# Epist/omnidirectional_collaborative_filtering

Measured on AMD Instinct MI355X. Metric: ratings/sec + masked-RMSE, ML-20M I-AutoRec at 1/2/4/8 MI355X, higher is better.
Workload: dtype f16

## Files before the change

include/ocf.h:

```cpp
#ifndef OCF_H_
#define OCF_H_
#include <stdint.h>

#ifdef __cplusplus
extern "C" {
#endif

#define OCF_DT_F32 0
#define OCF_DT_F16 1
#define OCF_DT_BF16 2

#define OCF_ACTV_LINEAR 0
#define OCF_ACTV_SIGMOID 1
#define OCF_ACTV_TANH 2
#define OCF_ACTV_RELU 3

#define OCF_OPTK_SGD 0
#define OCF_OPTK_ADAGRAD 1
#define OCF_OPTK_RMSPROP 2
#define OCF_OPTK_ADAM 3

#define OCF_EPI_SLAB 0
#define OCF_EPI_BIAS_ACT 1
#define OCF_EPI_GRAD_ACT 2
// ... 253 lines not shown
typedef struct OcfOptStepArgs {
  float* p; const void* g; int g_dtype; float* s1; float* s2; int64_t n; OcfOptParams opt;
  void* shadow; int shadow_dtype;
} OcfOptStepArgs;
int ocf_opt_step_ex(const OcfOptStepArgs* args, void* stream);

int ocf_bias_opt_from_partials(float* b, const float* db_part, int parts, int64_t ld, int n, float* s1, float* s2,
                               float* g_out, const OcfOptParams* opt, void* stream);

int ocf_sumsq(const float* x, int64_t n, float scale, float* ws, float* out, void* stream);

int ocf_stats_finalize(const float* stats_part, int n_parts, const float* row_sse_part, int n_tiles, int M,
                       float* out, void* stream);

#define OCF_LIVE_REC 144

typedef struct OcfTileBucketArgs {
  const int32_t* rows; const int64_t* rp; const int32_t* tptr; const int32_t* col; const int32_t* lidx;
  const int64_t* lboff;
  int krows, ntiles, gm, nk;
  int32_t* cnt; int32_t* bptr; int32_t* ent;
  int64_t cap;
  int counted; int32_t* cnt_clear;
  const uint8_t* rtag_in; const uint8_t* rtag_out; int rtag;
  uint8_t* live_in; uint8_t* live_out;
  int32_t* row_ptr; int32_t* row_ent;
} OcfTileBucketArgs;
int ocf_sparse_tiles(const OcfTileBucketArgs* args, void* stream);

typedef struct OcfRowListArgs {
  const int32_t* ecb; int64_t E;
  int32_t* col_cnt; int32_t* cursor; int n_cols;
  int32_t* row_ptr; int32_t* row_ent;
  const uint8_t* rtag_in; const uint8_t* rtag_out; int rtag;
  uint8_t* live_in; uint8_t* live_out;
} OcfRowListArgs;
int ocf_row_lists(const OcfRowListArgs* args, void* stream);

typedef struct OcfEpochRowListArgs {
  int n_sel; int B; int n_cols;
  const int32_t* rows;
  const int64_t* rp; const int32_t* col;
  const int64_t* lboff;
  const int32_t* sel;
  const int64_t* ebase;
  int32_t* cnt;
  int32_t* row_ptr;
  int32_t* row_ent;
  uint8_t* live;
  int n_rg;
  int64_t ebase0;
  int max_list;
  int64_t entries;
} OcfEpochRowListArgs;
int ocf_epoch_row_lists(const OcfEpochRowListArgs* args, void* stream);

typedef struct OcfRecipKeepArgs {
  uint32_t key[624]; int32_t pos;
  int32_t nb; int32_t B; int64_t n_entries;
  const int64_t* boff; const int64_t* ebase;
  double s0; double s1;
  uint8_t* keep;
  double* doubles;
  void* workspace; int64_t workspace_bytes;
} OcfRecipKeepArgs;
int64_t ocf_recip_keep_workspace(int nb, int B, int64_t n_entries, int pos);
int ocf_recip_keep(OcfRecipKeepArgs* args, void* stream);
int ocf_mt_host_random_sample(uint32_t* key, int32_t* pos, int64_t n, double* out);
int ocf_mt_host_jump(const uint32_t* key_in, int64_t n_blocks, uint32_t* key_out);

#define OCF_MAX_HIDDEN 8
typedef struct OcfModelDesc {
  int n_hidden;
  int N;
  int k_blocks;
  int hidden[OCF_MAX_HIDDEN];
  int act;
  float dropout;
  int compute_dtype;
  int max_batch;
  uint64_t seed;
  float* W[OCF_MAX_HIDDEN + 1];
  float* b[OCF_MAX_HIDDEN + 1];
} OcfModelDesc;
typedef struct OcfCtx OcfCtx;

int ocf_model_dims(const OcfModelDesc* desc, int64_t* rows, int64_t* cols);
int ocf_ctx_create(const OcfModelDesc* desc, OcfCtx** ctx);
int ocf_ctx_destroy(OcfCtx* ctx);
int ocf_forward(OcfCtx* ctx, const float* const* inputs, int64_t ld_in, int B, int training, uint64_t step,
                const float* out_mask, int64_t ld_mask, float* pred, int64_t ld_pred, uint8_t* const* masks_out,
                void* stream);
int ocf_masked_mse(const float* pred, const float* T, const float* out_mask, int64_t ld, int B, int N,
                   float* out_grad, int64_t ld_grad, float* out_stats, void* stream);
int ocf_backward(OcfCtx* ctx, const float* grad, int64_t ld_grad, int B, float gscale, float* const* gW,
                 float* const* gb, void* stream);

typedef struct OcfMlpStepArgs {
  int n_hidden;
  int B, Bp;
  int N, Np, k_blocks;
  int hidden[OCF_MAX_HIDDEN], hidden_p[OCF_MAX_HIDDEN];
  const float* x[3]; int64_t ld_x; const int64_t* rows;
  const float* out_mask; const float* targets; int64_t ld_t;
  float* W[OCF_MAX_HIDDEN + 1]; float* b[OCF_MAX_HIDDEN + 1];
  float* sW1[OCF_MAX_HIDDEN + 1]; float* sW2[OCF_MAX_HIDDEN + 1];
// ... 32 lines not shown
```

omnidirectional_collaborative_filtering_amd/_lib.py:

```python
from __future__ import annotations

import ctypes
import os

_HERE = os.path.dirname(os.path.abspath(__file__))
LIB_PATH = os.environ.get("OCF_LIB_PATH") or os.path.join(_HERE, "libocf.so")

DT_F32, DT_F16, DT_BF16 = 0, 1, 2
ACT = {"linear": 0, None: 0, "sigmoid": 1, "tanh": 2, "relu": 3}
OPT_SGD, OPT_ADAGRAD, OPT_RMSPROP, OPT_ADAM = 0, 1, 2, 3
LIVE_REC = 144
EPI_SLAB, EPI_BIAS_ACT, EPI_GRAD_ACT, EPI_GRAD, EPI_OPTIM, EPI_PREDICT, EPI_MASKED_MSE = range(7)

P = ctypes.c_void_p
I32 = ctypes.c_int
I64 = ctypes.c_int64
U64 = ctypes.c_uint64
F32 = ctypes.c_float


class OcfOptParams(ctypes.Structure):
    _fields_ = [("kind", I32), ("lr", F32), ("eps", F32), ("rho", F32), ("beta2", F32), ("l2", F32),
                ("gscale", F32)]


class OcfScatterArgs(ctypes.Structure):
    _fields_ = [
        ("rp1", P), ("col1", P), ("val1", P), ("dup1", P), ("rows1", P), ("keep1", P), ("boff1", P),
        ("s0", F32), ("s1", F32), ("seed", U64), ("stream", U64), ("mode", I32), ("pass_through", I32),
        ("rp2", P), ("col2", P), ("val2", P), ("dup2", P), ("rows2", P),
        ("B", I32), ("B_pad", I32), ("N", I32), ("aux", F32),
        ("X", P), ("Min", P), ("Mout", P), ("T", P), ("Mmiss", P), ("ld", I64),
        ("xin", P), ("xin_dtype", I32), ("xin_ld", I64), ("xin_block", I64), ("feed", I32), ("both", I32),
        ("tile_cnt", P), ("bk_ptr", P), ("bk_cur", P), ("bk_rc", P), ("bk_t", P), ("bk_m", P), ("n_tiles", I32),
        ("pos1", P),
        ("lboff1", P), ("lboff2", P), ("E1", I64), ("E2", I64), ("tflag1", P), ("tflag2", P),
        ("xin_clean", I32), ("xval1", P), ("tb_cnt", P), ("tb_nk", I32),
        ("rtag_in", P), ("rtag_out", P), ("rtag", I32), ("col_cnt", P), ("ecb", P),
    ]


class OcfRowListArgs(ctypes.Structure):
    _fields_ = [
        ("ecb", P), ("E", I64), ("col_cnt", P), ("cursor", P), ("n_cols", I32), ("row_ptr", P), ("row_ent", P),
        ("rtag_in", P), ("rtag_out", P), ("rtag", I32), ("live_in", P), ("live_out", P),
    ]


class OcfEpochScatterArgs(ctypes.Structure):
    _fields_ = [
        ("n_sel", I32), ("sel", P), ("ebase", P), ("max_e", I64), ("keep_off", P), ("stream_mul", U64),
        ("xval", P), ("tflag", P), ("ebase0", I64),
    ]


class OcfEpochRowListArgs(ctypes.Structure):
    _fields_ = [
        ("n_sel", I32), ("B", I32), ("n_cols", I32), ("rows", P), ("rp", P), ("col", P), ("lboff", P),
        ("sel", P), ("ebase", P), ("cnt", P), ("row_ptr", P), ("row_ent", P), ("live", P), ("n_rg", I32),
        ("ebase0", I64), ("max_list", I32), ("entries", I64),
    ]


class OcfEncTileArgs(ctypes.Structure):
    _fields_ = [
        ("rows", P), ("rp", P), ("tptr", P), ("tcol", P), ("tlidx", P), ("lboff", P), ("xval", P),
        ("W", P), ("ldw", I64), ("w_dtype", I32), ("B", I32), ("Bp", I32), ("n_tiles", I32), ("H", I32),
        ("splits", I32), ("part", P), ("nnz", I64), ("n_entries", I64), ("work", P), ("work_bytes", I64),
        ("max_row_len", I64),
    ]


class OcfGatherArgs(ctypes.Structure):
    _fields_ = [
        ("rows", P), ("rp", P), ("col", P), ("val", P), ("lboff", P), ("xval", P), ("flag", P),
        ("ch_row", P), ("ch_j0", P), ("ch_j1", P), ("n_chunks", I32),
        ("W", P), ("w_dtype", I32), ("ldw", I64), ("w_blocked", I32), ("H", I32), ("part", P),
        ("h", P), ("h_dtype", I32), ("bias", P), ("aux", F32), ("delta_e", P), ("chunk_stats", P),
        ("d_out", P), ("d_dtype", I32), ("ld_d", I64),
        ("enc_part", P), ("enc_cptr", P), ("bias_h", P), ("act", I32), ("keep", F32), ("seed", U64), ("stream", U64),
        ("a_out", P), ("mask_out", P), ("m_real", I32), ("n_real", I32), ("zero_word", P),
        ("jr", P), ("row_arrive", P),
    ]


REDUCE_RAW, REDUCE_BIAS_ACT, REDUCE_GRAD_ACT = 0, 1, 2


class OcfRowsReduceArgs(ctypes.Structure):
    _fields_ = [
        ("part", P), ("row_cptr", P), ("B", I32), ("Bp", I32), ("H", I32), ("mode", I32), ("out", P),
        ("bias", P), ("act", I32), ("keep", F32), ("seed", U64), ("stream", U64),
        ("mask_in", P), ("mask_out", P), ("a_out", P), ("a_in", P), ("h_out", P), ("h_dtype", I32), ("n_real", I32),
        ("db_part", P), ("gscale", F32), ("chunk_stats", P), ("stats_part", P), ("row_sse", P),
    ]


class OcfGemmArgs(ctypes.Structure):
    _fields_ = [
        ("compute_dtype", I32),
        ("A", P), ("a_dtype", I32), ("a_col", I32), ("lda", I64),
        ("B", P), ("b_dtype", I32), ("b_col", I32), ("ldb", I64),
        ("M", I32), ("N", I32), ("K", I32), ("splits", I32), ("order", I32), ("epi", I32),
        ("out", P), ("ld_out", I64), ("split_stride", I64),
        ("bias", P), ("act", I32), ("keep", F32), ("seed", U64), ("stream", U64),
        ("mask_in", P), ("mask_out", P), ("a_out", P), ("h_out", P), ("h_dtype", I32), ("a_in", P),
        ("db_part", P), ("ld_db", I64), ("m_real", I32), ("n_real", I32),
        ("p", P), ("s1", P), ("s2", P), ("opt", OcfOptParams),
        ("pmask", P), ("ld_pmask", I64),
        ("bk_ptr", P), ("bk_rc", P), ("bk_t", P), ("bk_m", P), ("stats_part", P), ("row_sse_part", P),
        ("t_rows", P), ("t_rp", P), ("t_tptr", P), ("t_col", P), ("t_val", P), ("t_lidx", P), ("t_flag", P),
        ("t_lboff", P), ("t_ntiles", I32), ("t_aux", F32),
        ("p_shadow", P), ("a_nt", I32), ("b_nt", I32), ("b_blocked", I32), ("shadow_blocked", I32),
# ... 228 lines not shown
```

omnidirectional_collaborative_filtering_amd/csrc/ocf_gemm.hip:

```cpp
#include <algorithm>
#include <cstdlib>
#include <type_traits>

#include "ocf_epilogues.h"
#include "ocf_internal.h"
#include "ocf_optim_ws.h"
#include "ocf_rows.h"

using namespace ocf;

namespace {

template <typename CT, bool ACOL, bool BCOL, typename BGT, class Epi, bool SPA = false>
void launch(const OcfGemmArgs& g, const typename Epi::Params& ep, hipStream_t s) {
  using Cfg = GemmCfg<CT, ACOL, BCOL, CT, BGT>;
  constexpr int LDS = std::max(Cfg::OPER_LDS, Epi::LDS_NEED);
  static_assert(LDS <= 160 * 1024, "LDS budget");
  GemmShape sh;
  sh.A = g.A; sh.B = g.B; sh.lda = g.lda; sh.ldb = g.ldb;
  sh.M = g.M; sh.N = g.N; sh.K = g.K; sh.order = g.order;
  sh.a_nt = g.a_nt != 0; sh.b_nt = g.b_nt != 0;
  sh.b_blk = g.b_blocked != 0;
  if (sh.b_blk)
    OCF_CHECK(sizeof(BGT) == 2 && g.ldb % 64 == 0, "ocf_gemm: blocked B needs a 16-bit compute-dtype B and ldb % 64 == 0");
// ... 206 lines not shown
}

}

extern "C" int ocf_set_tuning(const char* key, int value, int* previous) {
  OCF_TRY_BEGIN
  const std::string k = key ? key : "";
  if (k == "optim_rows") {
    if (previous) *previous = g_optim_rows;
    g_optim_rows = value ? 1 : 0;
  } else if (k == "rows_long") {
    if (previous) *previous = g_rows_long;
    g_rows_long = value < 0 ? -1 : (value ? 1 : 0);
  } else if (k == "rows_dual") {
    if (previous) *previous = g_rows_dual;
    g_rows_dual = value ? 1 : 0;
  } else if (k == "rows_dual_parts") {
    if (previous) *previous = g_rows_dual_parts;
    OCF_CHECK(value >= 0 && value <= 64, "ocf_set_tuning: rows_dual_parts 0 (by size) or 1..64");
    g_rows_dual_parts = value;
  } else if (k == "rows_dual_pf") {
    if (previous) *previous = g_rows_dual_pf;
    g_rows_dual_pf = value < 0 ? -1 : value ? 1 : 0;
  } else if (k == "rows_dual_large") {
    if (previous) *previous = g_rows_dual_large;
    g_rows_dual_large = value ? 1 : 0;
  } else if (k == "rows_dual_count") {
    if (previous) *previous = g_rows_dual_count;
    g_rows_dual_count = 0;
  } else if (k == "rows_small_waves") {
    if (previous) *previous = g_rows_small_waves;
    g_rows_small_waves = value;
  } else if (k == "optim_ws") {
    if (previous) *previous = optim_ws_on() ? 1 : 0;
    g_optim_ws = value ? 1 : 0;
  } else if (k == "pair_wait_polls") {
    if (previous) *previous = g_pair_wait_polls;
    OCF_CHECK(value > 0, "ocf_set_tuning: pair_wait_polls > 0");
    g_pair_wait_polls = value;
  } else if (k == "encdec_max_polls") {
    if (previous) *previous = g_encdec_max_polls;
    OCF_CHECK(value != 0, "ocf_set_tuning: encdec_max_polls != 0");
    g_encdec_max_polls = value;
  } else if (k == "encdec_rowres") {
    if (previous) *previous = g_encdec_rowres;
    if (value >= 0) g_encdec_rowres = value ? 1 : 0;
  } else if (k == "mlp_max_polls") {
    if (previous) *previous = g_mlp_max_polls;
    OCF_CHECK(value != 0, "ocf_set_tuning: mlp_max_polls != 0");
    g_mlp_max_polls = value;
  } else if (k == "enc_tiles_pack") {
    if (previous) *previous = g_enc_tiles_pack;
    g_enc_tiles_pack = value ? 1 : 0;
  } else if (k == "optim_ws_max_k") {
    if (previous) *previous = g_optim_ws_max_k;
    g_optim_ws_max_k = value;
  } else {
    throw std::runtime_error("ocf_set_tuning: unknown key '" + k + "'");
  }
  OCF_TRY_END
}

namespace {
void check_gemm(const OcfGemmArgs& g) {
  OCF_CHECK((g.A || g.a_sparse) && g.B, "ocf_gemm: null operand");
  OCF_CHECK(g.M > 0 && g.N > 0 && g.K > 0, "ocf_gemm: empty shape");
  OCF_CHECK(g.M % GT_BM == 0 && g.N % GT_BN == 0, "ocf_gemm: M and N must be multiples of 128");
  const int bk = g.compute_dtype == OCF_F32 ? 32 : 64;
  OCF_CHECK(g.K % bk == 0, "ocf_gemm: K must be a multiple of 64 (f16/bf16) or 32 (f32)");
  OCF_CHECK(g.a_dtype == g.compute_dtype, "ocf_gemm: A must be in the compute dtype");
  OCF_CHECK(g.lda % 8 == 0 && g.ldb % 8 == 0, "ocf_gemm: leading dimensions must be multiples of 8");
  OCF_CHECK(g.splits >= 1, "ocf_gemm: splits >= 1");
  OCF_CHECK(g.splits == 1 || g.epi == OCF_EPI_SLAB, "ocf_gemm: split-K only with the SLAB epilogue");
  if (g.a_sparse) {
    OCF_CHECK(g.a_col && (g.epi == OCF_EPI_OPTIM || g.epi == OCF_EPI_GRAD),
              "ocf_gemm: sparse A only for OPTIM / GRAD with a_col = 1");
    OCF_CHECK(g.sp_rows && g.sp_rp && g.sp_tptr && g.sp_col && g.sp_lidx && g.sp_lboff && g.sp_vals &&
                  g.sp_ntiles * GT_BM >= g.M && g.sp_krows <= g.K,
              "ocf_gemm: sparse A descriptor incomplete");
  }
  OCF_CHECK(!(g.cb_p || g.jb_part || g.js_sp) || (g.epi == OCF_EPI_OPTIM && g.a_col),
            "ocf_gemm: folded jobs only with OPTIM on [K][M] A");
  OCF_CHECK(!g.cb_p || g.sp_colsum, "ocf_gemm: cb_p needs sp_colsum");
  OCF_CHECK(!g.jb_part || g.jb_p, "ocf_gemm: jb_part needs jb_p");
  OCF_CHECK(!g.js_sp || g.js_out, "ocf_gemm: js_sp needs js_out");
}

}

extern "C" int ocf_gemm(const OcfGemmArgs* args, void* stream) {
  OCF_TRY_BEGIN
  const OcfGemmArgs& g = *args;
  check_gemm(g);
  hipStream_t s = (hipStream_t)stream;
  switch (g.compute_dtype) {
    case OCF_F16: dispatch<_Float16>(g, s); break;
    case OCF_BF16: dispatch<__bf16>(g, s); break;
    case OCF_F32: dispatch<float>(g, s); break;
    default: throw std::runtime_error("ocf_gemm: bad compute dtype");
  }
  OCF_TRY_END
}

extern "C" int ocf_gemm_pair(const OcfGemmArgs* a, const OcfGemmArgs* b, OcfPairSync* sync, void* stream) {
  OCF_TRY_BEGIN
  OCF_CHECK(a && b, "ocf_gemm_pair: null arguments");
// ... 55 lines not shown
```

omnidirectional_collaborative_filtering_amd/csrc/ocf_internal.h:

```cpp
#pragma once
#include <exception>
#include <stdexcept>
#include <string>

#include "../../include/ocf.h"
#include "ocf_common.h"

namespace ocf {
using ScatterArgs = OcfScatterArgs;
void set_error(const std::string& msg);
uint32_t* async_error_word();
void check_async_errors();
extern int g_mlp_max_polls;
extern int g_encdec_max_polls;
extern int g_encdec_rowres;
bool rank_rowres_enc(const OcfGatherArgs& e, const OcfRowsReduceArgs& r, hipStream_t s);
bool rank_rowres_dec(const OcfBiasActArgs& hb, const OcfGatherArgs& d, const OcfRowsReduceArgs& r, hipStream_t s);
extern int g_enc_tiles_pack;
uint32_t* encdec_gate_word();
uint32_t encdec_generation();
uint32_t next_encdec_generation();
}

#define OCF_TRY_BEGIN try { ocf::check_async_errors();
#define OCF_TRY_END                                       \
  return 0;                                               \
  }                                                       \
  catch (const std::exception& e) {                       \
    ocf::set_error(e.what());                             \
    return 1;                                             \
  }

#define OCF_CHECK(cond, msg)                              \
  do {                                                    \
    if (!(cond)) throw std::runtime_error(msg);           \
  } while (0)

#define OCF_HIP(expr)                                                               \
  do {                                                                              \
    hipError_t _e = (expr);                                                         \
    if (_e != hipSuccess)                                                           \
      throw std::runtime_error(std::string("HIP error: ") + hipGetErrorString(_e) + \
                               " at " __FILE__ ":" + std::to_string(__LINE__));     \
  } while (0)
```

omnidirectional_collaborative_filtering_amd/csrc/ocf_sparse.hip:

```cpp
#include <algorithm>
#include <cstdlib>

#include "ocf_epilogues.h"
#include "ocf_internal.h"

namespace ocf {

#ifndef OCF_RG_THREADS
#define OCF_RG_THREADS 256
#endif
constexpr int RG_THREADS = OCF_RG_THREADS;
constexpr int RG_MAX_H = 512;
#ifndef OCF_RG_U
#define OCF_RG_U 4
#endif
constexpr int RG_U = OCF_RG_U;
#ifndef OCF_RG_UE
#define OCF_RG_UE 4
#endif
constexpr int RG_UE = OCF_RG_UE;
#ifndef OCF_RG_UD
#define OCF_RG_UD 4
#endif
constexpr int RG_UD = OCF_RG_UD;
// ... 1680 lines not shown
    if (a.live) {
      uint8_t* rec = a.live + ((int64_t)s * (n_cols / 128) + t) * OCF_LIVE_REC;
      const int k = (w ? n0s : 0) + __popcll(bal & ((1ull << lane) - 1));
      if (n > 0) rec[16 + (k & 7) * 16 + (k >> 3)] = (uint8_t)tid;
      if (w == 1 && lane == 0) *reinterpret_cast<int*>(rec) = n0s + __popcll(bal);
    }
    if (n > ERL_MID) {
      int* q = erl_queue(a);
      const int qi = atomicAdd(q, 1);
      q[1 + 2 * qi] = s;
      q[2 + 2 * qi] = t * 128 + tid;
    } else if (n > 64) {
      mids[atomicAdd(&nmid, 1)] = tid;
    }
  }
  const int c0 = 8 * w;
  int mx = lane < 8 ? s_n[c0 + lane] : 0;
  if (mx > 64) mx = 0;
#pragma unroll
  for (int o = 4; o > 0; o >>= 1) mx = max(mx, __shfl_xor(mx, o, 64));
  mx = __shfl(mx, 0, 64);
  if (mx > 32) erl_wave_lists<64>(ent, s_lo, s_n, c0, lane);
  else if (mx > 16) erl_wave_lists<32>(ent, s_lo, s_n, c0, lane);
  else if (mx > 8) erl_wave_lists<16>(ent, s_lo, s_n, c0, lane);
  else if (mx > 1) erl_wave_lists<8>(ent, s_lo, s_n, c0, lane);
  __syncthreads();
  for (int q = 0; q < nmid; ++q) {
    const int c = mids[q], lq = s_lo[c], nq = s_n[c];
    for (int i = tid; i < nq; i += 1024) buf[i] = ent[lq + i];
    __syncthreads();
    wg_bitonic<1024>(buf, nq);
    for (int i = tid; i < nq; i += 1024) ent[lq + i] = buf[i];
    __syncthreads();
  }
}

__global__ void __launch_bounds__(1024) erl_sort_long_kernel(OcfEpochRowListArgs a) {
  __shared__ int2 buf[ERL_LONG_MAX];
  const int* q = erl_queue(a);
  const int nq = q[0];
  for (int qi = blockIdx.x; qi < nq; qi += gridDim.x) {
    const int s = q[1 + 2 * qi], m = q[2 + 2 * qi];
    const int* rp = a.row_ptr + (int64_t)s * (a.n_cols + 1);
    int2* ent = reinterpret_cast<int2*>(a.row_ent) + (a.ebase[s] - a.ebase0);
    const int lo = rp[m], n = rp[m + 1] - lo;
    for (int i = threadIdx.x; i < n; i += 1024) buf[i] = ent[lo + i];
    __syncthreads();
    wg_bitonic<1024>(buf, n);
    for (int i = threadIdx.x; i < n; i += 1024) ent[lo + i] = buf[i];
    __syncthreads();
  }
}

}

extern "C" int ocf_epoch_row_lists(const OcfEpochRowListArgs* args, void* stream) {
  OCF_TRY_BEGIN
  const OcfEpochRowListArgs& a = *args;
  OCF_CHECK(a.rows && a.rp && a.col && a.lboff && a.sel && a.ebase && a.cnt && a.row_ptr && a.row_ent,
            "ocf_epoch_row_lists: null pointer");
  OCF_CHECK(a.n_cols > 0 && a.n_cols % 128 == 0, "ocf_epoch_row_lists: n_cols > 0, % 128");
  OCF_CHECK(a.B > 0 && a.B <= ERL_MAXB, "ocf_epoch_row_lists: 0 < B <= 4096 (one entry per batch row and column)");
  OCF_CHECK(a.n_sel >= 0 && a.n_sel <= 65535, "ocf_epoch_row_lists: 0 <= n_sel <= 65535");
  OCF_CHECK(a.n_rg >= 0 && a.n_rg <= 64 && a.n_rg <= a.B, "ocf_epoch_row_lists: 0 <= n_rg <= min(64, B)");
  if (a.n_sel == 0) return 0;
  hipStream_t s = (hipStream_t)stream;
  const int cb = erl_block_cols(a.B), ncb = (a.n_cols + cb - 1) / cb;
  const size_t lds = erl_lds_bytes(a.B);
  static const bool lds_attr = [] {
    return hipFuncSetAttribute((const void*)erl_count_kernel, hipFuncAttributeMaxDynamicSharedMemorySize, ERL_LDS) ==
               hipSuccess &&
           hipFuncSetAttribute((const void*)erl_fill_kernel, hipFuncAttributeMaxDynamicSharedMemorySize, ERL_LDS) ==
               hipSuccess;
  }();
  OCF_CHECK(lds_attr, "ocf_epoch_row_lists: cannot raise the dynamic LDS limit");
  const int nrg = a.n_rg > 1 ? a.n_rg : 1;
  hipLaunchKernelGGL(erl_count_kernel, dim3(ncb, a.n_sel, nrg), dim3(ERL_THREADS), lds, s, a, cb);
  const int nsb = (a.n_cols + ERL_SB - 1) / ERL_SB;
  if (nsb == 1) {
    hipLaunchKernelGGL(erl_gsum_kernel<true>, dim3(1, a.n_sel), dim3(1024), 0, s, a);
  } else {
    hipLaunchKernelGGL(erl_gsum_kernel<false>, dim3(nsb, a.n_sel), dim3(1024), 0, s, a);
    hipLaunchKernelGGL(erl_scan_kernel, dim3(nsb, a.n_sel), dim3(1024), 0, s, a);
  }
  if (OCF_ERL_XCD) {
    const int64_t T = (int64_t)ncb * a.n_sel * nrg;
    hipLaunchKernelGGL(erl_fill_kernel, dim3((unsigned)((T + 7) / 8 * 8)), dim3(ERL_THREADS), lds, s, a, cb);
  } else {
    hipLaunchKernelGGL(erl_fill_kernel, dim3(ncb, a.n_sel, nrg), dim3(ERL_THREADS), lds, s, a, cb);
  }
  if (a.entries >= 4 * (int64_t)a.n_sel * a.n_cols)
    hipLaunchKernelGGL(erl_sort_wave_kernel, dim3(a.n_cols / 128, a.n_sel), dim3(1024), 0, s, a);
  else
    hipLaunchKernelGGL(erl_sort_kernel, dim3(a.n_cols / 128, a.n_sel), dim3(128), 0, s, a);
  if (a.max_list <= 0 || a.max_list > ERL_MID)
    hipLaunchKernelGGL(erl_sort_long_kernel, dim3(64), dim3(1024), 0, s, a);
  OCF_HIP(hipGetLastError());
  OCF_TRY_END
}

extern "C" int ocf_row_lists(const OcfRowListArgs* args, void* stream) {
  OCF_TRY_BEGIN
  const OcfRowListArgs& a = *args;
  OCF_CHECK(a.ecb && a.col_cnt && a.cursor && a.row_ptr && a.row_ent, "ocf_row_lists: null pointer");
  OCF_CHECK(a.n_cols > 0 && a.n_cols % 128 == 0 && a.n_cols <= (1 << 19), "ocf_row_lists: 0 < n_cols <= 2^19, % 128");
  OCF_CHECK((!a.live_in || a.rtag_in) && (!a.live_out || a.rtag_out), "ocf_row_lists: live records need row tags");
  OCF_CHECK(!(a.live_in || a.live_out) || (a.rtag >= 1 && a.rtag <= 255), "ocf_row_lists: 1 <= rtag <= 255");
  hipStream_t s = (hipStream_t)stream;
  hipLaunchKernelGGL(rl_scan_kernel, dim3((a.n_cols + RL_CHUNK - 1) / RL_CHUNK), dim3(1024), 0, s, a);
  if (a.E > 0) hipLaunchKernelGGL(rl_fill_kernel, dim3((unsigned)((a.E + 255) / 256)), dim3(256), 0, s, a);
  hipLaunchKernelGGL(rl_sort_kernel, dim3(a.n_cols / 128), dim3(128), 0, s, a);
  hipLaunchKernelGGL(rl_sort_long_kernel, dim3(RL_LONG_BLOCKS), dim3(256), 0, s, a);
  OCF_HIP(hipGetLastError());
  OCF_TRY_END
}

extern "C" int ocf_sparse_tiles(const OcfTileBucketArgs* args, void* stream) {
  OCF_TRY_BEGIN
  const OcfTileBucketArgs& a = *args;
// ... 23 lines not shown
```

omnidirectional_collaborative_filtering_amd/data_reader.py:

```python
from __future__ import annotations

import ctypes
import os
import time

import numpy as np
import torch

from . import _lib
from .dataset import FixedSplit, load_reference_json
from .engine import TILE, cur_stream, ptr, ru
from .parallel import shard_batches

AUX_FEED = {None: 0, "dropout": 1, "both": 1, "causal": 2, "zeros": 3}
GATHER_CHUNK = 256
GATHER_CHUNK_SMALL = 64
GATHER_CHUNK_MID = 96
GATHER_CHUNK_MID_MIN_CHUNKS = 512
GATHER_BIG = 100_000
ROWLIST_MAX_BATCHES = 4096
ROWLIST_MAX_ENTRIES = 4096
ROWLIST_RG_WORK = 160
ROWS_DENSE_MAX_COLS = 170 * 128


_RNG_STREAMS = {}


def _h2d(x, dev):
    t = torch.as_tensor(np.ascontiguousarray(x))
    if torch.device(dev).type != "cuda":
        return t.to(dev)
    return t.pin_memory().to(dev, non_blocking=True)


def _rng_stream(dev):
    key = torch.device(dev).index if torch.device(dev).index is not None else torch.cuda.current_device()
    if key not in _RNG_STREAMS:
        _RNG_STREAMS[key] = torch.cuda.Stream(device=key)
    return _RNG_STREAMS[key]


class _DeviceCSR:
    def __init__(self, csr, dev):
        self.host = csr
        self.rp = torch.as_tensor(csr.row_ptr, device=dev)
        self.col = torch.as_tensor(csr.col, device=dev)
        self.val = torch.as_tensor(csr.val, device=dev)
        self.dup = None if csr.dup is None else torch.as_tensor(csr.dup, device=dev)
        self.pos = None if csr.pos is None else torch.as_tensor(csr.pos, device=dev)
        self.lens = csr.row_lengths()
        self.rng_lens = csr.rng_lengths()
        self.dev = dev
        self._tiles = {}

    def tiles(self, n_cols):
        if n_cols not in self._tiles:
            col_s, val_s, lidx_s, tptr = self.host.tile_index(n_cols)
            d = self.dev
            self._tiles[n_cols] = dict(t_col=torch.as_tensor(col_s, device=d), t_val=torch.as_tensor(val_s, device=d),
                                       t_lidx=torch.as_tensor(lidx_s, device=d), t_tptr=torch.as_tensor(tptr, device=d),
                                       t_ntiles=tptr.shape[1] - 1,
                                       t_maxlen=int(self.lens.max()) if len(self.lens) else 0)
        return self._tiles[n_cols]


class data_reader(object):

    def __init__(self, num_items, num_users, filepath=None, nonsequentialusers=False, use_json=True,
                 eval_mode="ablation", useTimestamps=False, reverse_user_item_data=False, dataset=None,
                 rng="numpy", device=None):
        if useTimestamps:
            raise NotImplementedError("useTimestamps: broken in the reference (data_reader.py:358-359 feeds the "
                                      "whole dict); not supported")
        if eval_mode != "fixed_split":
            raise NotImplementedError("eval_mode='ablation' (split_for_validation) is out of scope; use fixed_split")
        self.num_items = int(num_items)
        self.num_users = int(num_users)
        self.filepath = filepath
        self.nonsequentialusers = nonsequentialusers
        self.eval_mode = eval_mode
        self.useTimestamps = False
        self.rng = rng
        if dataset is None:
            dataset = load_reference_json(filepath, reverse_user_item_data, use_json)
        elif isinstance(dataset, str):
            dataset = FixedSplit.load(dataset)
        self.data = dataset
        if dataset.num_cols != self.num_items:
            raise ValueError("num_items=%d but the data has %d columns" % (self.num_items, dataset.num_cols))
        self.items_to_densevec = {c: i for i, c in enumerate(dataset.col_ids)}
        self.densevec_to_items = {i: c for i, c in enumerate(dataset.col_ids)}
        self.train_set = list(dataset.train.keys)
        self.val_set = list(dataset.valid_tgt.keys)
        self.test_set = list(dataset.test_tgt.keys)
        self.train_set_size = len(self.train_set)
        self.val_set_size = len(self.val_set)
        self.test_set_size = len(self.test_set)
        self.device = torch.device(device if device is not None else "cuda")
        self._dev = None
        print("Finished loading data")

    def _on_device(self):
        if self._dev is None:
            d = self.device
            self._dev = {k: _DeviceCSR(getattr(self.data, k), d)
                         for k in ("train", "valid_in", "valid_tgt", "test_in", "test_tgt")}
        return self._dev

    def split_for_validation(self, val_split, seed=None):
        raise NotImplementedError("ablation eval mode is out of scope")

    def data_gen(self, batch_size, data_sparsity, train_val_test="train", shuffle=True,
                 auxilliary_mask_type="dropout", aux_var_value=-1, return_target_count=False,
                 sparse_representation=False, pass_through_input_training=False):
        if sparse_representation:
            raise NotImplementedError("sparse_representation needs a patched Keras backend in the reference "
# ... 131 lines not shown
        out = {}
        for key, src, ch, lb in (("enc", self.src1, self.chunks1, self.lboff1_dev),
                                 ("dec", self.src1 if self.src2 is None else self.src2, self.chunks2,
                                  self.lboff1_dev if self.src2 is None else self.lboff2_dev)):
            c0 = int(ch["cbase"][bi])
            out[key] = dict(rows=self.rows_dev.data_ptr() + 4 * bi * B, rp=ptr(src.rp), col=ptr(src.col),
                            val=ptr(src.val), lboff=lb.data_ptr() + 8 * bi * (B + 1),
                            ch_row=ch["ch_row"].data_ptr() + 4 * c0, ch_j0=ch["ch_j0"].data_ptr() + 4 * c0,
                            ch_j1=ch["ch_j1"].data_ptr() + 4 * c0, n_chunks=int(ch["cbase"][bi + 1]) - c0,
                            row_cptr=ch["row_cptr"].data_ptr() + 4 * bi * (B + 1),
                            max_chunks=int(ch["max_chunks"][bi]))
        if self.split == "train":
            out["row_lists"] = lambda n_cols, bi=bi: self.row_lists(bi, n_cols)
            N = self.r.num_items
            out["rows_dense"] = bool(self.num_batches and self.nnz1.mean() >= 2 * N and N <= ROWS_DENSE_MAX_COLS)
        return out

    def prepare_row_lists(self, n_cols, batches=None):
        t0 = time.perf_counter()
        if not self.started:
            self._start()
        if self.split != "train":
            raise ValueError("row lists are built for train batches (inputs = targets)")
        nb = self.num_batches
        if batches is None:
            batches = shard_batches(nb, *self.dp_shard) if self.dp_shard else np.arange(nb)
        if isinstance(batches, (list, tuple, range)):
            sel = np.array(sorted(set(batches)), dtype=np.int64)
        else:
            sel = np.asarray(batches, dtype=np.int64)
            if sel.size > 1 and not bool((sel[1:] > sel[:-1]).all()):
                sel = np.unique(sel)
        if len(sel) and (sel[0] < 0 or sel[-1] >= nb):
            raise ValueError("batch index out of range")
        cap = int(min(ROWLIST_MAX_BATCHES, max(1, (1 << 28) // (n_cols + 1))))
        if len(sel) > cap:
            sel = sel[:cap]
        if self.src1.dup is not None and len(sel):
            self._check_list_lengths(sel)
        dev = self.rows_dev.device
        ep = self._epoch_tables(dev)
        n = len(sel)
        if n and int(sel[-1]) - int(sel[0]) + 1 == n:
            b0 = int(sel[0])
            e0 = int(ep["ebase"][b0])
            ebase = ep["ebase"][b0:b0 + n + 1] - e0
            p_sel, p_ebase = ep["sel_dev"].data_ptr() + 4 * b0, ep["ebase_dev"].data_ptr() + 8 * b0
        else:
            e0 = 0
            ebase = np.zeros(n + 1, dtype=np.int64)
            np.cumsum(self.nnz1[sel], out=ebase[1:])
            p_ebase, p_sel = self._stage([ebase, sel.astype(np.int32)], dev)
        E = int(ebase[-1])
        n_rg = int(min(8, max(1, -(-ROWLIST_RG_WORK // max(n, 1)))))
        need = (("cnt", n_rg * n * n_cols // 2 + n * (n_cols // 4096 + 1) + 1 + 2 * (E // 1025 + 1), torch.int32),
                ("row_ptr", n * (n_cols + 1), torch.int32), ("row_ent", 2 * max(E, 1), torch.int32),
                ("live", max(n * (n_cols // 128) * _lib.LIVE_REC, 1), torch.uint8),
                ("xval", max(E, 1), torch.float32), ("tflag", max(E, 1), torch.uint8))
        bufs = getattr(self, "_rl_bufs", None)
        if bufs is None:
            bufs = self._rl_bufs = {}
        for k, m, dt in need:
            b = bufs.get(k)
            if b is None or b[1] < m:
                t = torch.empty(m, dtype=dt, device=dev)
                bufs[k] = (t, m, t.data_ptr())
        t1 = time.perf_counter()
        a = _lib.OcfEpochRowListArgs()
        a.n_sel, a.B, a.n_cols, a.n_rg, a.ebase0 = n, self.B, n_cols, n_rg, e0
        a.max_list = self.B if self.src1.dup is None else 0
        a.entries = E
        a.rows, a.rp, a.col, a.lboff = ep["args_const"]
        a.sel, a.ebase = p_sel, p_ebase
        a.cnt, a.row_ptr, a.row_ent, a.live = bufs["cnt"][2], bufs["row_ptr"][2], bufs["row_ent"][2], bufs["live"][2]
        _lib.call("ocf_epoch_row_lists", a, cur_stream())
        t2 = time.perf_counter()
        if n:
            es = _lib.OcfEpochScatterArgs()
            es.keep_off = ep["keep_off"]
            es.n_sel, es.sel, es.ebase, es.ebase0 = n, p_sel, p_ebase, e0
            es.max_e = int(self.nnz1[sel].max())
            es.stream_mul = 2
            es.xval, es.tflag = bufs["xval"][2], bufs["tflag"][2]
            _lib.call("ocf_epoch_scatter", ep["scatter_base"], es, cur_stream())
        self._rl = dict(row_ptr=bufs["row_ptr"][0], row_ent=bufs["row_ent"][0], live=bufs["live"][0],
                        xval=bufs["xval"][0], tflag=bufs["tflag"][0], n_cols=n_cols,
                        slot=dict(zip(sel.tolist(), range(n))), ebase_host=ebase, fields={})
        t3 = time.perf_counter()
        self.rl_host_us = dict(plan=(t1 - t0) * 1e6, lists=(t2 - t1) * 1e6, scatter=(t3 - t2) * 1e6)

    def _epoch_tables(self, dev):
        ep = getattr(self, "_ep_tabs", None)
        if ep is None:
            nb = self.num_batches
            ebase = np.zeros(nb + 1, dtype=np.int64)
            np.cumsum(self.nnz1, out=ebase[1:])
            ep = dict(ebase=ebase, ebase_dev=_h2d(ebase, dev), sel_dev=_h2d(np.arange(max(nb, 1), dtype=np.int32), dev),
                      scatter_base=self.scatter_args(0) if nb else _lib.OcfScatterArgs(),
                      args_const=(ptr(self.rows_dev), ptr(self.src1.rp), ptr(self.src1.col), ptr(self.lboff1_dev)))
            ep["keep_off_dev"] = None if self.keep_dev is None else \
                _h2d(np.ascontiguousarray(self.keep_off, dtype=np.int64), dev)
            ep["keep_off"] = None if ep["keep_off_dev"] is None else ep["keep_off_dev"].data_ptr()
            self._ep_tabs = ep
        return ep

    def _stage(self, parts, dev):
        sizes = [(a.nbytes + 7) // 8 * 8 for a in parts]
        tot = max(sum(sizes), 8)
        if torch.device(dev).type != "cuda":
            flat = np.zeros(tot, dtype=np.uint8)
        st = getattr(self, "_stage_bufs", None)
        if torch.device(dev).type == "cuda":
            if st is None or st[0].numel() < tot:
                st = [torch.empty(2 * tot, dtype=torch.uint8, pin_memory=True),
                      torch.empty(2 * tot, dtype=torch.uint8, device=dev), None]
                self._stage_bufs = st
            if st[2] is not None:
                st[2].synchronize()
            flat = st[0].numpy()
        off, addr = 0, []
        for a, sz in zip(parts, sizes):
            flat[off:off + a.nbytes] = np.ascontiguousarray(a).view(np.uint8).ravel()
            addr.append(off)
            off += sz
        if torch.device(dev).type != "cuda":
            self._stage_bufs = [None, torch.as_tensor(flat), None]
            return [self._stage_bufs[1].data_ptr() + o for o in addr]
# ... 147 lines not shown
```

Before: 443.5 million.

## Add one-pass epoch row-list kernel using a precomputed per-row column-block index

Precomputes, once per column count, a per-source-row index of entries sorted by column and bucketed into 4096-column blocks. A new single-pass kernel then builds each batch's transposed row lists per column block in LDS: counting, scanning, scattering and segment-sorting there, and writing the live records as well. This replaces the multi-kernel row-list construction for sparse batches and trades a one-time device sort plus extra index memory for lower per-epoch list-building cost. It also clamps n_rg to B.

Result: no change. 445.0 million, median of 6 (+0.3%).

```diff
diff --git a/include/ocf.h b/include/ocf.h
--- a/include/ocf.h
+++ b/include/ocf.h
@@ -329,6 +329,8 @@
   int64_t ebase0;
   int max_list;
   int64_t entries;
+  const int32_t* blk_off; const int32_t* blk_ent;
+  int blk_w; int n_blk;
 } OcfEpochRowListArgs;
 int ocf_epoch_row_lists(const OcfEpochRowListArgs* args, void* stream);
 
diff --git a/omnidirectional_collaborative_filtering_amd/_lib.py b/omnidirectional_collaborative_filtering_amd/_lib.py
--- a/omnidirectional_collaborative_filtering_amd/_lib.py
+++ b/omnidirectional_collaborative_filtering_amd/_lib.py
@@ -59,6 +59,7 @@
         ("n_sel", I32), ("B", I32), ("n_cols", I32), ("rows", P), ("rp", P), ("col", P), ("lboff", P),
         ("sel", P), ("ebase", P), ("cnt", P), ("row_ptr", P), ("row_ent", P), ("live", P), ("n_rg", I32),
         ("ebase0", I64), ("max_list", I32), ("entries", I64),
+        ("blk_off", P), ("blk_ent", P), ("blk_w", I32), ("n_blk", I32),
     ]
 
 
diff --git a/omnidirectional_collaborative_filtering_amd/csrc/ocf_gemm.hip b/omnidirectional_collaborative_filtering_amd/csrc/ocf_gemm.hip
--- a/omnidirectional_collaborative_filtering_amd/csrc/ocf_gemm.hip
+++ b/omnidirectional_collaborative_filtering_amd/csrc/ocf_gemm.hip
@@ -282,6 +282,17 @@
   } else if (k == "enc_tiles_pack") {
     if (previous) *previous = g_enc_tiles_pack;
     g_enc_tiles_pack = value ? 1 : 0;
+  } else if (k == "erl_onepass") {
+    if (previous) *previous = g_erl_onepass;
+    OCF_CHECK(value == 0 || value == 1, "ocf_set_tuning: erl_onepass 0 or 1");
+    g_erl_onepass = value;
+  } else if (k == "erl_onepass_mean") {
+    if (previous) *previous = g_erl_onepass_mean;
+    OCF_CHECK(value >= 0, "ocf_set_tuning: erl_onepass_mean >= 0");
+    g_erl_onepass_mean = value;
+  } else if (k == "erl_onepass_count") {
+    if (previous) *previous = g_erl_onepass_count;
+    g_erl_onepass_count = 0;
   } else if (k == "optim_ws_max_k") {
     if (previous) *previous = g_optim_ws_max_k;
     g_optim_ws_max_k = value;
diff --git a/omnidirectional_collaborative_filtering_amd/csrc/ocf_internal.h b/omnidirectional_collaborative_filtering_amd/csrc/ocf_internal.h
--- a/omnidirectional_collaborative_filtering_amd/csrc/ocf_internal.h
+++ b/omnidirectional_collaborative_filtering_amd/csrc/ocf_internal.h
@@ -17,6 +17,9 @@
 bool rank_rowres_enc(const OcfGatherArgs& e, const OcfRowsReduceArgs& r, hipStream_t s);
 bool rank_rowres_dec(const OcfBiasActArgs& hb, const OcfGatherArgs& d, const OcfRowsReduceArgs& r, hipStream_t s);
 extern int g_enc_tiles_pack;
+extern int g_erl_onepass;
+extern int g_erl_onepass_mean;
+extern int g_erl_onepass_count;
 uint32_t* encdec_gate_word();
 uint32_t encdec_generation();
 uint32_t next_encdec_generation();
diff --git a/omnidirectional_collaborative_filtering_amd/csrc/ocf_sparse.hip b/omnidirectional_collaborative_filtering_amd/csrc/ocf_sparse.hip
--- a/omnidirectional_collaborative_filtering_amd/csrc/ocf_sparse.hip
+++ b/omnidirectional_collaborative_filtering_amd/csrc/ocf_sparse.hip
@@ -1756,6 +1756,249 @@
   }
 }
 
+constexpr int ERL1_THREADS = 512;
+constexpr int ERL1_WAVES = ERL1_THREADS / 64;
+constexpr int ERL1_U = 16;
+constexpr int ERL1_CAP_MAX = ERL1_THREADS * ERL1_U;
+constexpr int ERL1_REG = 16;
+constexpr int ERL_OB_MAX = 4096;
+constexpr int ERL1_LDS_TWO = 76 * 1024;
+constexpr int ERL1_LDS_ONE = 156 * 1024;
+int g_erl_onepass = 1;
+int g_erl_onepass_count = 0;
+int g_erl_onepass_mean = 4;
+
+inline int64_t erl1_fixed_bytes(int B, int w) { return (int64_t)B * 20 + 8 + (int64_t)w * 4; }
+inline int erl1_cap(int B, int w, int max_list, size_t* lds) {
+  int64_t cap = (ERL1_LDS_TWO - erl1_fixed_bytes(B, w)) / 8;
+  if (cap < max_list || cap < 1024) cap = (ERL1_LDS_ONE - erl1_fixed_bytes(B, w)) / 8;
+  cap = std::min<int64_t>(cap, ERL1_CAP_MAX);
+  if (lds) *lds = (size_t)(erl1_fixed_bytes(B, w) + cap * 8);
+  return (int)cap;
+}
+
+__device__ __forceinline__ int erl1_sum(int v, int* wred) {
+#pragma unroll
+  for (int o = 32; o > 0; o >>= 1) v += __shfl_xor(v, o, 64);
+  __syncthreads();
+  if ((threadIdx.x & 63) == 0) wred[threadIdx.x >> 6] = v;
+  __syncthreads();
+  int t = 0;
+#pragma unroll
+  for (int k = 0; k < ERL1_WAVES; ++k) t += wred[k];
+  return t;
+}
+
+__device__ __forceinline__ int erl1_scan(int* x, int n, int* wred) {
+  const int tid = threadIdx.x, lane = tid & 63, w = tid >> 6;
+  const int per = (n + ERL1_THREADS - 1) / ERL1_THREADS, i0 = tid * per, i1 = min(n, i0 + per);
+  __syncthreads();
+  int sum = 0;
+  for (int i = i0; i < i1; ++i) sum += x[i];
+  const int incl = wave_incl_scan(sum, lane);
+  if (lane == 63) wred[w] = incl;
+  __syncthreads();
+  int off = 0, tot = 0;
+#pragma unroll
+  for (int k = 0; k < ERL1_WAVES; ++k) {
+    const int v = wred[k];
+    off += k < w ? v : 0;
+    tot += v;
+  }
+  int run = off + incl - sum;
+  for (int i = i0; i < i1; ++i) {
+    const int v = x[i];
+    x[i] = run;
+    run += v;
+  }
+  __syncthreads();
+  return tot;
+}
+
+__device__ __forceinline__ int erl1_lower(const int2* ce, int p, int q, int c) {
+  while (p < q) {
+    const int m = (p + q) >> 1;
+    if (ce[m].x < c) p = m + 1;
+    else q = m;
+  }
+  return p;
+}
+
+__global__ void __launch_bounds__(ERL1_THREADS, 4) erl_onepass_kernel(OcfEpochRowListArgs a, int cap) {
+  extern __shared__ int64_t erl1_dyn[];
+  __shared__ uint32_t nz[ERL_OB_MAX / 32];
+  __shared__ int wred[ERL1_WAVES];
+  __shared__ int mids[ERL1_CAP_MAX / (ERL1_REG + 1) + 1];
+  __shared__ int nmid;
+  const int tid = threadIdx.x, lane = tid & 63, w = tid >> 6;
+  const int k = blockIdx.x, s = blockIdx.y, B = a.B, W = a.blk_w;
+  const int c0 = k * W, nc = min(W, a.n_cols - c0), cend = c0 + nc;
+  int64_t* rbase = erl1_dyn;
+  int2* img = reinterpret_cast<int2*>(rbase + B);
+  int* lb = reinterpret_cast<int*>(img + cap);
+  int* slo = lb + B;
+  int* pre = slo + B;
+  int* cnt = pre + B + 1;
+  const int bi = a.sel[s];
+  const int64_t* lbo = a.lboff + (int64_t)bi * (B + 1);
+  const int32_t* rows = a.rows + (int64_t)bi * B;
+  const int nbo = a.n_blk + 1;
+  const int2* bent = reinterpret_cast<const int2*>(a.blk_ent);
+  int* rp = a.row_ptr + (int64_t)s * (a.n_cols + 1);
+  int2* ent = reinterpret_cast<int2*>(a.row_ent) + (a.ebase[s] - a.ebase0);
+
+  for (int i = tid; i < ERL_OB_MAX / 32; i += ERL1_THREADS) nz[i] = 0u;
+  int bsum = 0;
+  for (int b = tid; b < B; b += ERL1_THREADS) {
+    const int r = rows[b];
+    int o0 = 0, o1 = 0;
+    int64_t rb = 0;
+    if (r >= 0) {
+      rb = a.rp[r];
+      const int32_t* bo = a.blk_off + (int64_t)r * nbo + k;
+      o0 = bo[0];
+      o1 = bo[1];
+    }
+    rbase[b] = rb;
+    lb[b] = (int)lbo[b];
+    slo[b] = o0;
+    pre[b] = o1 - o0;
+    bsum += o0;
+  }
+  int base = erl1_sum(bsum, wred);
+
+  int lo = c0, hi = cend;
+  bool whole = true;
+  while (lo < cend) {
+    if (!whole) {
+      for (int b = tid; b < B; b += ERL1_THREADS) {
+        const int r = rows[b];
+        int p0 = 0, p1 = 0;
+        if (r >= 0) {
+          const int32_t* bo = a.blk_off + (int64_t)r * nbo + k;
+          const int2* ce = bent + rbase[b];
+          p0 = erl1_lower(ce, bo[0], bo[1], lo);
+          p1 = erl1_lower(ce, p0, bo[1], hi);
+        }
+        slo[b] = p0;
+        pre[b] = p1 - p0;
+      }
+    }
+    whole = false;
+    const int total = erl1_scan(pre, B, wred);
+    const int wd = hi - lo;
+    if (total > cap) {
+      if (wd <= 1) break;
+      hi = lo + wd / 2;
+      continue;
+    }
+    if (tid == 0) {
+      pre[B] = total;
+      nmid = 0;
+    }
+    for (int i = tid; i < wd; i += ERL1_THREADS) cnt[i] = 0;
+    __syncthreads();
+
+    uint16_t* own = reinterpret_cast<uint16_t*>(img);
+    for (int b = w; b < B; b += ERL1_WAVES) {
+      const int p0 = pre[b], n = pre[b + 1] - p0;
+      for (int j = lane; j < n; j += 64) own[p0 + j] = (uint16_t)b;
+    }
+    __syncthreads();
+    int key[ERL1_U], ev[ERL1_U];
+#pragma unroll
+    for (int u = 0; u < ERL1_U; ++u) {
+      const int i = tid + u * ERL1_THREADS;
+      key[u] = -1;
+      ev[u] = 0;
+      if (i < total) {
+        const int p = own[i];
+        const int2 ce = bent[rbase[p] + slo[p] + (i - pre[p])];
+        const int c = ce.x - lo;
+        if ((unsigned)c < (unsigned)wd) {
+          key[u] = c | (p << 16);
+          ev[u] = lb[p] + ce.y;
+        }
+      }
+    }
+#pragma unroll
+    for (int u = 0; u < ERL1_U; ++u)
+      if (key[u] >= 0) atomicAdd(&cnt[key[u] & 0xFFFF], 1);
+    __syncthreads();
+    for (int i = tid; i < wd; i += ERL1_THREADS)
+      if (cnt[i] > 0) atomicOr(&nz[(lo - c0 + i) >> 5], 1u << ((lo - c0 + i) & 31));
+    erl1_scan(cnt, wd, wred);
+    for (int i = tid; i < wd; i += ERL1_THREADS) rp[lo + i] = base + cnt[i];
+    if (hi == a.n_cols && tid == 0) rp[a.n_cols] = base + total;
+    __syncthreads();
+#pragma unroll
+    for (int u = 0; u < ERL1_U; ++u)
+      if (key[u] >= 0) {
+        const int pos = atomicAdd(&cnt[key[u] & 0xFFFF], 1);
+        if (pos < cap) img[pos] = make_int2(ev[u], key[u] >> 16);
+      }
+    __syncthreads();
+
+    for (int i0 = 0; i0 < wd; i0 += ERL1_THREADS) {
+      const int i = i0 + tid;
+      int l0 = 0, n = 0;
+      if (i < wd) {
+        l0 = i ? cnt[i - 1] : 0;
+        n = cnt[i] - l0;
+      }
+      int nm = n <= ERL1_REG ? n : 0;
+#pragma unroll
+      for (int off = 32; off > 0; off >>= 1) nm = max(nm, __shfl_xor(nm, off, 64));
+      if (n > 1 && n <= ERL1_REG) {
+        if (nm <= 4) rl_reg_sort<4>(img + l0, n);
+        else if (nm <= 8) rl_reg_sort<8>(img + l0, n);
+        else rl_reg_sort<ERL1_REG>(img + l0, n);
+      } else if (n > ERL1_REG) {
+        mids[atomicAdd(&nmid, 1)] = i;
+      }
+    }
+    __syncthreads();
+    const int nq = nmid;
+    for (int q = w; q < nq; q += ERL1_WAVES) {
+      const int i = mids[q], l0 = i ? cnt[i - 1] : 0, n = cnt[i] - l0;
+      if (n <= 64) {
+        int2 v = lane < n ? img[l0 + lane] : make_int2(0x7fffffff, 0);
+        v = seg_bitonic<64>(v, lane);
+        if (lane < n) img[l0 + lane] = v;
+      }
+    }
+    __syncthreads();
+    for (int q = 0; q < nq; ++q) {
+      const int i = mids[q], l0 = i ? cnt[i - 1] : 0, n = cnt[i] - l0;
+      if (n > 64) wg_bitonic<ERL1_THREADS>(img + l0, n);
+    }
+    for (int i = tid; i < total; i += ERL1_THREADS) ent[base + i] = img[i];
+    __syncthreads();
+    base += total;
+    lo = hi;
+    hi = min(cend, lo + 2 * wd);
+  }
+
+  if (a.live) {
+    __syncthreads();
+    for (int i = tid; i < nc; i += ERL1_THREADS) {
+      const int t = i >> 7, j = i & 127, jw = j >> 5;
+      uint8_t* rec = a.live + ((int64_t)s * (a.n_cols / 128) + (c0 >> 7) + t) * OCF_LIVE_REC;
+      int kk = 0, L = 0;
+#pragma unroll
+      for (int x = 0; x < 4; ++x) {
+        const int pc = __popc(nz[4 * t + x]);
+        kk += x < jw ? pc : 0;
+        L += pc;
+      }
+      const uint32_t word = nz[4 * t + jw];
+      kk += __popc(word & ((1u << (j & 31)) - 1u));
+      if ((word >> (j & 31)) & 1u) rec[16 + (kk & 7) * 16 + (kk >> 3)] = (uint8_t)j;
+      if (j == 0) *reinterpret_cast<int*>(rec) = L;
+    }
+  }
+}
+
 }
 
 extern "C" int ocf_epoch_row_lists(const OcfEpochRowListArgs* args, void* stream) {
@@ -1769,6 +2012,25 @@
   OCF_CHECK(a.n_rg >= 0 && a.n_rg <= 64 && a.n_rg <= a.B, "ocf_epoch_row_lists: 0 <= n_rg <= min(64, B)");
   if (a.n_sel == 0) return 0;
   hipStream_t s = (hipStream_t)stream;
+  if (a.blk_off && a.blk_ent && g_erl_onepass) {
+    OCF_CHECK(a.blk_w >= 128 && a.blk_w <= ERL_OB_MAX && a.blk_w % 128 == 0,
+              "ocf_epoch_row_lists: blk_w a multiple of 128, <= 4096");
+    OCF_CHECK(a.n_blk == (a.n_cols + a.blk_w - 1) / a.blk_w, "ocf_epoch_row_lists: n_blk = ceil(n_cols / blk_w)");
+    size_t lds1 = 0;
+    const int cap = erl1_cap(a.B, a.blk_w, a.max_list, &lds1);
+    const bool sparse = g_erl_onepass_mean <= 0 ||
+                        (a.entries > 0 && a.entries < (int64_t)g_erl_onepass_mean * a.n_sel * a.n_cols);
+    if (a.max_list > 0 && a.max_list <= cap && sparse) {
+      static const bool lds1_attr = hipFuncSetAttribute((const void*)erl_onepass_kernel,
+                                                        hipFuncAttributeMaxDynamicSharedMemorySize,
+                                                        ERL1_LDS_ONE) == hipSuccess;
+      OCF_CHECK(lds1_attr, "ocf_epoch_row_lists: cannot raise the dynamic LDS limit");
+      hipLaunchKernelGGL(erl_onepass_kernel, dim3(a.n_blk, a.n_sel), dim3(ERL1_THREADS), lds1, s, a, cap);
+      OCF_HIP(hipGetLastError());
+      ++g_erl_onepass_count;
+      return 0;
+    }
+  }
   const int cb = erl_block_cols(a.B), ncb = (a.n_cols + cb - 1) / cb;
   const size_t lds = erl_lds_bytes(a.B);
   static const bool lds_attr = [] {
diff --git a/omnidirectional_collaborative_filtering_amd/data_reader.py b/omnidirectional_collaborative_filtering_amd/data_reader.py
--- a/omnidirectional_collaborative_filtering_amd/data_reader.py
+++ b/omnidirectional_collaborative_filtering_amd/data_reader.py
@@ -21,6 +21,7 @@
 ROWLIST_MAX_BATCHES = 4096
 ROWLIST_MAX_ENTRIES = 4096
 ROWLIST_RG_WORK = 160
+ROWLIST_BLOCK_COLS = 4096
 ROWS_DENSE_MAX_COLS = 170 * 128
 
 
@@ -53,6 +54,7 @@
         self.rng_lens = csr.rng_lengths()
         self.dev = dev
         self._tiles = {}
+        self._blocks = {}
 
     def tiles(self, n_cols):
         if n_cols not in self._tiles:
@@ -63,6 +65,27 @@
                                        t_ntiles=tptr.shape[1] - 1,
                                        t_maxlen=int(self.lens.max()) if len(self.lens) else 0)
         return self._tiles[n_cols]
+
+    def block_index(self, n_cols, width=None):
+        width = ROWLIST_BLOCK_COLS if width is None else width
+        key = (int(n_cols), int(width))
+        if key not in self._blocks:
+            n_rows, nblk = len(self.lens), -(-int(n_cols) // width)
+            d = self.col.device
+            rows = torch.repeat_interleave(torch.arange(n_rows, dtype=torch.int64, device=d),
+                                           torch.as_tensor(self.lens, dtype=torch.int64, device=d))
+            skey, order = torch.sort(rows * int(n_cols) + self.col.to(torch.int64), stable=True)
+            del rows
+            srow = torch.div(skey, int(n_cols), rounding_mode="floor")
+            scol = skey - srow * int(n_cols)
+            del skey
+            ent = torch.stack([scol, order - self.rp.to(torch.int64)[srow]], dim=1).to(torch.int32).contiguous()
+            del order
+            cnt = torch.bincount(srow * nblk + torch.div(scol, width, rounding_mode="floor"), minlength=n_rows * nblk)
+            off = torch.zeros((n_rows, nblk + 1), dtype=torch.int32, device=d)
+            off[:, 1:] = torch.cumsum(cnt.view(n_rows, nblk), dim=1)
+            self._blocks[key] = dict(blk_ent=ent, blk_off=off, blk_w=int(width), n_blk=nblk)
+        return self._blocks[key]
 
 
 class data_reader(object):
@@ -300,7 +323,7 @@
             np.cumsum(self.nnz1[sel], out=ebase[1:])
             p_ebase, p_sel = self._stage([ebase, sel.astype(np.int32)], dev)
         E = int(ebase[-1])
-        n_rg = int(min(8, max(1, -(-ROWLIST_RG_WORK // max(n, 1)))))
+        n_rg = int(min(8, self.B, max(1, -(-ROWLIST_RG_WORK // max(n, 1)))))
         need = (("cnt", n_rg * n * n_cols // 2 + n * (n_cols // 4096 + 1) + 1 + 2 * (E // 1025 + 1), torch.int32),
                 ("row_ptr", n * (n_cols + 1), torch.int32), ("row_ent", 2 * max(E, 1), torch.int32),
                 ("live", max(n * (n_cols // 128) * _lib.LIVE_REC, 1), torch.uint8),
@@ -321,6 +344,9 @@
         a.rows, a.rp, a.col, a.lboff = ep["args_const"]
         a.sel, a.ebase = p_sel, p_ebase
         a.cnt, a.row_ptr, a.row_ent, a.live = bufs["cnt"][2], bufs["row_ptr"][2], bufs["row_ent"][2], bufs["live"][2]
+        if n and a.max_list > 0:
+            bx = self.src1.block_index(n_cols)
+            a.blk_off, a.blk_ent, a.blk_w, a.n_blk = ptr(bx["blk_off"]), ptr(bx["blk_ent"]), bx["blk_w"], bx["n_blk"]
         _lib.call("ocf_epoch_row_lists", a, cur_stream())
         t2 = time.perf_counter()
         if n:
```
